# OpenDrift/opendrift

Measured on NVIDIA H100. Metric: particle-steps/sec (RK4, 10M particles/GPU, 512x512x50 field), higher is better.
Workload: dtype f64

## Files before the change

include/odcuda.h:

```cpp
#ifndef ODCUDA_H
#define ODCUDA_H

#include <stdint.h>

#ifdef __cplusplus
extern "C" {
#endif

typedef struct od_ctx od_ctx;

enum od_status {
    OD_OK = 0,
    OD_ERR_CUDA = -1,
    OD_ERR_ARG = -2,
    OD_ERR_STATE = -3,
    OD_ERR_NOMEM = -4
};

enum od_scheme { OD_EULER = 0, OD_RK2 = 1, OD_RK4 = 2 };

enum od_time_mode {
    OD_T_LERP = 0,
    OD_T_FIRST = 1,
    OD_T_SECOND = 2,
// ... 8 lines not shown
                       OD_INTERP_NEAREST = 32  };

#define OD_MAX_LEVELS 128
#define OD_ABI_VERSION 1

int od_abi_version(void);

int od_create(int device, od_ctx** out);
void od_destroy(od_ctx* ctx);
const char* od_last_error(od_ctx* ctx);
int od_set_stream(od_ctx* ctx, void* cuda_stream);
int od_sync(od_ctx* ctx);
enum od_option { OD_OPT_TILE = 1, OD_OPT_SPEC = 2 };
int od_set_option(od_ctx* ctx, int option, int value);
int od_device_sm_count(od_ctx* ctx);

#define OD_PROJ_STERE_SPHERE 1
#define OD_PROJ_MERC 2
#define OD_PROJ_LCC 3
#define OD_PROJ_STERE_ELLPS 4
#define OD_PROJ_OB_TRAN 5
typedef struct od_proj_desc {
    int32_t kind;
    int32_t has_lat_ts;
    double a;
    double lat_0, lon_0, lat_ts;
    double k_0, x_0, y_0;
    double es;
    double lat_1, lat_2;
} od_proj_desc;

typedef struct od_group_desc {
    int32_t ncomp;
    int32_t nx, ny, nz;
    int32_t lon_mode;
    int32_t n_slots;
    int32_t wrap_x;
    int32_t global_x;
    double x0, xspan, y0, yspan;
    double xmin, xmax, ymin, ymax;
    float fallback[2];
    od_proj_desc proj;
    int32_t rotate_vectors;
    int32_t pad_;
} od_group_desc;

#define OD_MAX_GROUPS 64
int od_group_define(od_ctx* ctx, int group, const od_group_desc* desc, const double* h_z_levels);
int od_group_free(od_ctx* ctx, int group);
int od_group_upload(od_ctx* ctx, int group, int slot, int comp, const float* src, int src_is_device);
int od_group_fill_nan(od_ctx* ctx, int group, int slot, int comp, int max_iterations, int64_t* h_remaining);
int od_group_slot_ptr(od_ctx* ctx, int group, int slot, int comp, float** d_out);
int od_group_touch(od_ctx* ctx, int group, int slot);
int od_group_set_window(od_ctx* ctx, int group, const od_group_desc* window);
int od_bbox(od_ctx* ctx, int64_t n, const double* d_lon, const double* d_lat, double* h_out4);
int od_group_set_fallback(od_ctx* ctx, int group, float fallback0, float fallback1);

typedef struct od_time_sample {
    int32_t slot_a, slot_b;
    int32_t mode;
    int32_t pad_;
    double w;
} od_time_sample;

int od_interp(od_ctx* ctx, int group, const od_time_sample* ts, int64_t n,
              const double* d_lon, const double* d_lat, const void* d_z, int flags,
              void* d_out0, void* d_out1);

int od_geod_fwd(od_ctx* ctx, int64_t n, double* d_lon, double* d_lat,
                const double* d_az_deg, const double* d_dist_m);

int od_update_positions(od_ctx* ctx, int64_t n, double* d_lon, double* d_lat,
                        const void* d_xvel, const void* d_yvel, int vel_f64,
                        const int32_t* d_moving, double dt);

#define OD_MATH_EXACT 0
#define OD_MATH_FAST 1
#define OD_MATH_SERIES 2

typedef struct od_advect_args {
    int32_t scheme;
    int32_t group_uv;
    od_time_sample t_start;
    od_time_sample t_mid;
    od_time_sample t_end;
    double dt;
    int64_t n;
    double* d_lon;
    double* d_lat;
    const void* d_z;
    const void* d_factor;
    int32_t factor_f64;
    int32_t pos_f32;
    const int32_t* d_moving;
    const float* d_k1_u;
    const float* d_k1_v;
    double truncate_below;
    float* d_env_u;
    float* d_env_v;
    int32_t z_f64;
    int32_t pad3_;
    const double* d_noise_cur;
    int32_t noise_kinds;
    int32_t fast;
    int32_t n_chain;
    int32_t chain_group[2];
// ... 335 lines not shown
```

opendrift_b200/_lib.py:

```python
import ctypes as C
import os

_HERE = os.path.dirname(os.path.abspath(__file__))
LIB_PATH = os.environ.get('ODCUDA_LIB') or os.path.join(_HERE, 'libodcuda.so')

OD_EULER, OD_RK2, OD_RK4 = 0, 1, 2
OD_T_LERP, OD_T_FIRST, OD_T_SECOND, OD_T_MISSING = 0, 1, 2, 3
OD_LON_0_360, OD_LON_PM180 = 0, 1
OD_OPT_TILE = 1
OD_OPT_SPEC = 2
OD_MATH_EXACT, OD_MATH_FAST, OD_MATH_SERIES = 0, 1, 2
OD_MIX_ENVIRONMENT, OD_MIX_LARGE1994, OD_MIX_SUNDBY1983, OD_MIX_CONSTANT = 0, 1, 2, 3
OD_MAX_LEVELS = 128
OD_MAX_GROUPS = 64
OD_MAX_CHAIN = 2
SCHEMES = {'euler': OD_EULER, 'runge-kutta': OD_RK2, 'runge-kutta4': OD_RK4}


class ProjDesc(C.Structure):
    _fields_ = [('kind', C.c_int32), ('has_lat_ts', C.c_int32), ('a', C.c_double), ('lat_0', C.c_double),
                ('lon_0', C.c_double), ('lat_ts', C.c_double), ('k_0', C.c_double), ('x_0', C.c_double), ('y_0', C.c_double),
                ('es', C.c_double), ('lat_1', C.c_double), ('lat_2', C.c_double)]


# ... 102 lines not shown
                ('d_sea_floor', C.c_void_p), ('d_status', C.c_void_p), ('d_moving', C.c_void_p), ('dt', C.c_double),
                ('sea_surface_height', C.c_float), ('z_f64', C.c_int32), ('tv_f64', C.c_int32), ('seafloor_code', C.c_int32),
                ('h_n_deactivated', C.POINTER(C.c_int64))]


class BookkeepArgs(C.Structure):
    _fields_ = [('n', C.c_int64), ('d_lon', C.c_void_p), ('d_lat', C.c_void_p), ('d_z', C.c_void_p), ('d_age', C.c_void_p),
                ('d_status', C.c_void_p), ('d_moving', C.c_void_p), ('d_ids', C.c_void_p), ('dt_age', C.c_double),
                ('max_age', C.c_double), ('west', C.c_double), ('east', C.c_double), ('south', C.c_double), ('north', C.c_double),
                ('outside_code', C.c_int32), ('retired_code', C.c_int32), ('z_f64', C.c_int32), ('age_f64', C.c_int32),
                ('pos_f32', C.c_int32), ('only_deactivated', C.c_int32), ('n_total', C.c_int64), ('col', C.c_int32), ('ncols', C.c_int32),
                ('d_buf_lon', C.c_void_p), ('d_buf_lat', C.c_void_p), ('d_buf_z', C.c_void_p), ('d_buf_status', C.c_void_p),
                ('h_counts', C.POINTER(C.c_int64))]


class CoastArgs(C.Structure):
    _fields_ = [('n', C.c_int64), ('d_mask', C.c_void_p), ('d_lon', C.c_void_p), ('d_lat', C.c_void_p), ('d_z', C.c_void_p),
                ('d_age', C.c_void_p), ('d_status', C.c_void_p), ('d_moving', C.c_void_p), ('d_ids', C.c_void_p),
                ('d_prev_lon', C.c_void_p), ('d_prev_lat', C.c_void_p), ('n_total', C.c_int64), ('id_base', C.c_int32),
                ('action', C.c_int32), ('ssh', C.c_float), ('stranded_code', C.c_int32), ('seeded_code', C.c_int32), ('missing_code', C.c_int32),
                ('check_seeded', C.c_int32), ('z_f64', C.c_int32), ('age_f64', C.c_int32), ('h_counts', C.POINTER(C.c_int64))]


OD_INTERP_POS_F32, OD_INTERP_NO_FALLBACK, OD_INTERP_Z_F64, OD_INTERP_NO_ROTATE, OD_INTERP_OUT_F64, OD_INTERP_NEAREST = 1, 2, 4, 8, 16, 32
OD_PACK_MAX_COLS, OD_PACK_MAX_WORLD = 16, 64


class PackArgs(C.Structure):
    _fields_ = [('n', C.c_int64), ('d_lon', C.c_void_p), ('h_bounds', C.POINTER(C.c_double)), ('world', C.c_int32), ('ncols', C.c_int32),
                ('d_cols', C.c_void_p * OD_PACK_MAX_COLS), ('col_bytes', C.c_int32 * OD_PACK_MAX_COLS), ('rec_bytes', C.c_int32),
                ('pad_', C.c_int32), ('d_records', C.c_void_p), ('d_perm', C.c_void_p), ('h_counts', C.POINTER(C.c_int64))]


OD_PROJ_STERE_SPHERE = 1
OD_PROJ_MERC, OD_PROJ_LCC, OD_PROJ_STERE_ELLPS, OD_PROJ_OB_TRAN = 2, 3, 4, 5
OD_ANALYTIC_DOUBLE_GYRE = 1

_P = C.c_void_p
SYMBOLS = {
    'od_abi_version': (C.c_int, []),
    'od_create': (C.c_int, [C.c_int, C.POINTER(_P)]),
    'od_destroy': (None, [_P]),
    'od_last_error': (C.c_char_p, [_P]),
    'od_set_stream': (C.c_int, [_P, _P]),
    'od_sync': (C.c_int, [_P]),
    'od_set_option': (C.c_int, [_P, C.c_int, C.c_int]),
    'od_device_sm_count': (C.c_int, [_P]),
    'od_group_define': (C.c_int, [_P, C.c_int, C.POINTER(GroupDesc), C.POINTER(C.c_double)]),
    'od_group_free': (C.c_int, [_P, C.c_int]),
    'od_group_upload': (C.c_int, [_P, C.c_int, C.c_int, C.c_int, _P, C.c_int]),
    'od_group_fill_nan': (C.c_int, [_P, C.c_int, C.c_int, C.c_int, C.c_int, C.POINTER(C.c_int64)]),
    'od_group_slot_ptr': (C.c_int, [_P, C.c_int, C.c_int, C.c_int, C.POINTER(_P)]),
    'od_group_touch': (C.c_int, [_P, C.c_int, C.c_int]),
    'od_group_set_fallback': (C.c_int, [_P, C.c_int, C.c_float, C.c_float]),
    'od_group_set_window': (C.c_int, [_P, C.c_int, C.POINTER(GroupDesc)]),
    'od_bbox': (C.c_int, [_P, C.c_int64, _P, _P, C.POINTER(C.c_double)]),
    'od_interp': (C.c_int, [_P, C.c_int, C.POINTER(TimeSample), C.c_int64, _P, _P, _P, C.c_int, _P, _P]),
    'od_geod_fwd': (C.c_int, [_P, C.c_int64, _P, _P, _P, _P]),
    'od_update_positions': (C.c_int, [_P, C.c_int64, _P, _P, _P, _P, C.c_int, _P, C.c_double]),
    'od_advect_current': (C.c_int, [_P, C.POINTER(AdvectArgs)]),
    'od_advect_current_host': (C.c_int, [_P, C.POINTER(AdvectArgs), C.POINTER(HostIO)]),
    'od_step_oceandrift_host': (C.c_int, [_P, C.POINTER(StepArgs), C.POINTER(HostIO)]),
    'od_step_oceandrift': (C.c_int, [_P, C.POINTER(StepArgs)]),
    'od_leeway_step': (C.c_int, [_P, C.POINTER(LeewayArgs)]),
    'od_analytic_interp': (C.c_int, [_P, C.POINTER(AnalyticDesc), C.c_double, C.c_int64, _P, _P, C.c_int, _P, _P]),
    'od_history_scatter': (C.c_int, [_P, C.POINTER(HistoryArgs)]),
    'od_analytic_advect': (C.c_int, [_P, C.POINTER(AnalyticDesc), C.POINTER(AnalyticAdvectArgs)]),
    'od_minmax_f32': (C.c_int, [_P, C.c_int64, _P, _P, C.POINTER(C.c_float), C.POINTER(C.c_float)]),
    'od_stokes_drift': (C.c_int, [_P, C.POINTER(StokesArgs)]),
    'od_stokes_parameterised': (C.c_int, [_P, C.c_int64, _P, _P, _P, C.c_int32, _P, C.c_int32, _P, _P, _P]),
    'od_vertical_mixing': (C.c_int, [_P, C.POINTER(MixArgs)]),
    'od_vertical_mixing_settle': (C.c_int, [_P, C.POINTER(MixArgs), _P, _P, C.POINTER(C.c_int64)]),
    'od_resuspend': (C.c_int, [_P, C.c_int64, _P, _P, C.c_float, _P, _P, C.c_int32]),
    'od_ship_step': (C.c_int, [_P, C.c_int64, _P, _P, _P, _P, _P, _P, _P, _P, _P, C.c_int32, C.c_int32, C.c_int32, C.c_int32, C.c_int32,
                               C.c_int32, C.c_float, C.c_int32, C.c_double, C.POINTER(C.c_int32)]),
    'od_plast_step': (C.c_int, [_P, C.c_int64, _P, _P, _P, _P, C.c_int32, _P, _P, _P, C.c_int32, _P, _P, C.c_uint64, C.c_int32, _P, C.c_int32,
                                C.c_int32, _P, _P, _P, C.c_int32, C.c_double, C.c_double, C.POINTER(C.c_int32)]),
    'od_larval_develop': (C.c_int, [_P, C.c_int64, _P, _P, _P, C.c_int32, _P, C.c_int32, _P, C.c_int32, _P, C.c_int32, _P, C.c_int32, _P,
                                    C.c_int32, C.c_int32, _P, C.c_double, C.POINTER(C.c_int32)]),
    'od_larval_migrate': (C.c_int, [_P, C.c_int64, _P, C.c_int32, _P, C.c_int32, _P, C.c_int32, C.c_double, C.c_double, C.c_double]),
    'od_vertical_buoyancy': (C.c_int, [_P, C.POINTER(BuoyancyArgs)]),
    'od_bookkeeping': (C.c_int, [_P, C.POINTER(BookkeepArgs)]),
    'od_coastline': (C.c_int, [_P, C.POINTER(CoastArgs)]),
    'od_store_previous': (C.c_int, [_P, C.c_int64, _P, _P, _P, C.c_int32, C.c_int64, _P, _P]),
    'od_store_previous_env': (C.c_int, [_P, C.c_int64, _P, _P, _P, C.c_int32, C.c_double, C.c_int32, C.c_int64, _P, _P]),
    'od_vertical_advection_corrected': (C.c_int, [_P, C.c_int64, _P, C.c_int32, _P, _P, _P, _P, C.c_float, _P, C.c_int32,
                                                  C.c_double]),
    'od_pack_by_owner': (C.c_int, [_P, C.POINTER(PackArgs)]),
    'od_unpack_records': (C.c_int, [_P, C.c_int64, _P, C.c_int32, C.POINTER(_P), C.POINTER(C.c_int32), C.c_int32]),
    'od_sort_by_cell': (C.c_int, [_P, C.c_int, C.c_int64, _P, _P, _P, _P]),
    'od_partition_active': (C.c_int, [_P, C.c_int64, _P, _P, C.POINTER(C.c_int64)]),
    'od_permute': (C.c_int, [_P, C.c_int64, _P, _P, _P, C.c_int]),
    'od_unpermute': (C.c_int, [_P, C.c_int64, _P, _P, _P, C.c_int]),
    'od_launch_count': (C.c_int64, [_P]),
}

_lib = None


def load():
    global _lib
    if _lib is not None:
        return _lib
    if not os.path.exists(LIB_PATH):
        raise RuntimeError(
            'opendrift_b200: %s is missing. This package has no CPU fallback; build the CUDA '
# ... 12 lines not shown
```

opendrift_b200/csrc/od_ctx.cuh:

```cuda
#pragma once
#include <cuda.h>
#include <cuda_runtime.h>
#include <stdint.h>
#include <string>
#include <vector>

#include "../../include/odcuda.h"
#include "od_advect.cuh"
#include "od_analytic.cuh"

using namespace od;

#define OD_PAIR_CACHE 4
#ifndef OD_BLOCK
#define OD_BLOCK 128
#endif
#ifndef OD_STEP_MINB
#define OD_STEP_MINB 8
#endif
#ifndef OD_SPEC_MINB
#define OD_SPEC_MINB 6
#endif

#define OD_TILE_BX 48
#define OD_TILE_BY 8
#define OD_TILE_BZ 2
#define OD_TILE_HALO 2

struct PairEntry {
    CUtensorMap tmap;
    bool tmap_ok = false;
    float* tex = nullptr;
    int slot_a = -1, slot_b = -1;
    uint64_t ver_a = 0, ver_b = 0;
    uint64_t last_use = 0;
};

struct Group {
    bool defined = false;
    od_group_desc desc;
    std::vector<float*> slots;
    std::vector<uint64_t> version;
    double* d_zs = nullptr;
    double* d_zy = nullptr;
    double* d_zl = nullptr;
    double* d_mxs = nullptr;
    double* d_mxy = nullptr;
    std::vector<double> h_levels;
    double zmin = 0, zmax = 0;
    PairEntry pairs[OD_PAIR_CACHE];
    size_t capacity = 0;
    size_t cells() const { return (size_t)desc.nx * desc.ny * desc.nz; }
};

struct od_ctx {
    int device = 0;
    cudaStream_t stream = nullptr;
    std::string err;
    Group groups[OD_MAX_GROUPS];
    int64_t launches = 0;
    uint64_t tick = 0;
    int sm_count = 0;
    int32_t* d_keys = nullptr;
    int32_t* d_bins = nullptr;
    int64_t keys_cap = 0, bins_cap = 0;
    int32_t* d_tilesums = nullptr;
    int64_t tiles_cap = 0;
    unsigned* d_red = nullptr;
    unsigned long long* d_bbox = nullptr;
    unsigned* d_cnt = nullptr;
    float* d_fill = nullptr;
    unsigned* d_fillcnt = nullptr;
    int coop_fill_blocks = -1;
    int64_t fill_cap = 0;
    int tile = 0;
    int spec = 1;
    cudaStream_t hstream[3] = {nullptr, nullptr, nullptr};
    cudaEvent_t hready = nullptr;
    char* hbuf = nullptr;
    int64_t hbuf_cap = 0;
};

static inline int fail(od_ctx* c, int code, const char* what, cudaError_t e = cudaSuccess) {
    if (c) {
        c->err = what;
        if (e != cudaSuccess) {
            c->err += ": ";
            c->err += cudaGetErrorString(e);
// ... 32 lines not shown
```

opendrift_b200/csrc/od_kernels.cu:

```cuda
#include <cuda.h>
#include <cuda_runtime.h>
#include <cooperative_groups.h>
#include <stdint.h>
#include <stdio.h>
#include <stdlib.h>
#include <string.h>
#include <string>
#include <vector>

#include "../../include/odcuda.h"
#include "od_advect.cuh"
#include "od_mix.cuh"
#include "od_stokes.cuh"
#include "od_leeway.cuh"
#include "od_ship.cuh"
#include "od_plast.cuh"
#include "od_larval.cuh"
#include "od_analytic.cuh"
#include "od_history.cuh"
#include "od_bookkeep.cuh"
#include "od_sealevel.cuh"
#include "od_ctx.cuh"

extern "C" int od_abi_version(void) { return OD_ABI_VERSION; }

extern "C" int od_create(int device, od_ctx** out) {
    if (!out) return OD_ERR_ARG;
    *out = nullptr;
    int count = 0;
    if (cudaGetDeviceCount(&count) != cudaSuccess || device < 0 || device >= count) return OD_ERR_CUDA;
    if (cudaSetDevice(device) != cudaSuccess) return OD_ERR_CUDA;
    od_ctx* c = new od_ctx();
    c->device = device;
    cudaDeviceGetAttribute(&c->sm_count, cudaDevAttrMultiProcessorCount, device);
    *out = c;
    return OD_OK;
}

static void free_group(Group& g) {
    for (float* p : g.slots) if (p) cudaFree(p);
    g.slots.clear();
    g.version.clear();
    if (g.d_zs) cudaFree(g.d_zs);
    if (g.d_zy) cudaFree(g.d_zy);
    if (g.d_zl) cudaFree(g.d_zl);
    if (g.d_mxs) cudaFree(g.d_mxs);
    if (g.d_mxy) cudaFree(g.d_mxy);
    g.d_zs = g.d_zy = g.d_zl = g.d_mxs = g.d_mxy = nullptr;
    g.h_levels.clear();
    for (auto& p : g.pairs) {
        if (p.tex) cudaFree(p.tex);
        p = PairEntry();
    }
    g.defined = false;
}

extern "C" void od_destroy(od_ctx* ctx) {
    if (!ctx) return;
    cudaSetDevice(ctx->device);
    for (auto& g : ctx->groups) free_group(g);
    if (ctx->d_keys) cudaFree(ctx->d_keys);
    if (ctx->d_bins) cudaFree(ctx->d_bins);
    if (ctx->d_red) cudaFree(ctx->d_red);
    if (ctx->d_bbox) cudaFree(ctx->d_bbox);
    if (ctx->d_cnt) cudaFree(ctx->d_cnt);
    if (ctx->d_fill) cudaFree(ctx->d_fill);
    if (ctx->d_fillcnt) cudaFree(ctx->d_fillcnt);
    if (ctx->d_tilesums) cudaFree(ctx->d_tilesums);
    if (ctx->hbuf) cudaFree(ctx->hbuf);
    for (int k = 0; k < 3; ++k)
        if (ctx->hstream[k]) cudaStreamDestroy(ctx->hstream[k]);
    if (ctx->hready) cudaEventDestroy(ctx->hready);
    delete ctx;
}

extern "C" const char* od_last_error(od_ctx* ctx) { return ctx ? ctx->err.c_str() : "null context"; }

extern "C" int od_set_stream(od_ctx* ctx, void* s) {
    if (!ctx) return OD_ERR_ARG;
    ctx->stream = (cudaStream_t)s;
    return OD_OK;
}

extern "C" int od_set_option(od_ctx* ctx, int option, int value) {
    if (!ctx) return OD_ERR_ARG;
    if (option == OD_OPT_TILE) { ctx->tile = value ? 1 : 0; return OD_OK; }
    if (option == OD_OPT_SPEC) { ctx->spec = value ? 1 : 0; return OD_OK; }
    return fail(ctx, OD_ERR_ARG, "od_set_option: unknown option");
}

extern "C" int od_sync(od_ctx* ctx) {
    if (!ctx) return OD_ERR_ARG;
    CK(cudaStreamSynchronize(ctx->stream));
    return OD_OK;
}

extern "C" int od_device_sm_count(od_ctx* ctx) { return ctx ? ctx->sm_count : 0; }
extern "C" int64_t od_launch_count(od_ctx* ctx) { return ctx ? ctx->launches : 0; }

extern "C" int od_group_define(od_ctx* ctx, int group, const od_group_desc* d, const double* h_z) {
    if (!ctx || !d || group < 0 || group >= OD_MAX_GROUPS) return fail(ctx, OD_ERR_ARG, "od_group_define: bad group");
    if (d->ncomp < 1 || d->ncomp > 2 || d->nx < 2 || d->ny < 2 || d->nz < 1 || d->nz > OD_MAX_LEVELS ||
        d->n_slots < 2 || d->n_slots > 64)
        return fail(ctx, OD_ERR_ARG, "od_group_define: bad shape");
// ... 260 lines not shown
        }
        if (still) atomicAdd(&cnt[it + 1], still);
        grid.sync();
        for (int64_t i = first; i < cells; i += stride) a[i] = tmp[i];
        grid.sync();
    }
}

__global__ void __launch_bounds__(OD_BLOCK) pack_pair2_kernel(const float* __restrict__ a0, const float* __restrict__ a1,
                                                               const float* __restrict__ b0, const float* __restrict__ b1,
                                                               float4* __restrict__ tex, int64_t cells) {
    int64_t i = (int64_t)blockIdx.x * blockDim.x + threadIdx.x;
    const int64_t stride = (int64_t)gridDim.x * blockDim.x;
    for (; i < cells; i += stride) tex[i] = make_float4(a0[i], a1[i], b0[i], b1[i]);
}

__global__ void __launch_bounds__(OD_BLOCK) pack_pair1_kernel(const float* __restrict__ a0, const float* __restrict__ b0,
                                                               float2* __restrict__ tex, int64_t cells) {
    int64_t i = (int64_t)blockIdx.x * blockDim.x + threadIdx.x;
    const int64_t stride = (int64_t)gridDim.x * blockDim.x;
    for (; i < cells; i += stride) tex[i] = make_float2(a0[i], b0[i]);
}

typedef CUresult (*od_encode_tiled_fn)(CUtensorMap*, CUtensorMapDataType, cuuint32_t, void*, const cuuint64_t*, const cuuint64_t*,
                                       const cuuint32_t*, const cuuint32_t*, CUtensorMapInterleave, CUtensorMapSwizzle,
                                       CUtensorMapL2promotion, CUtensorMapFloatOOBfill);

static od_encode_tiled_fn tensor_map_encoder() {
    static od_encode_tiled_fn fn = nullptr;
    static bool tried = false;
    if (!tried) {
        tried = true;
        void* f = nullptr;
        cudaDriverEntryPointQueryResult q;
        if (cudaGetDriverEntryPoint("cuTensorMapEncodeTiled", &f, cudaEnableDefault, &q) == cudaSuccess &&
            q == cudaDriverEntryPointSuccess)
            fn = (od_encode_tiled_fn)f;
    }
    return fn;
}

static bool make_tensor_map(const Group& g, float* tex, CUtensorMap* out) {
    od_encode_tiled_fn enc = tensor_map_encoder();
    if (!enc || g.desc.ncomp != 2) return false;
    const cuuint64_t dims[4] = {4, (cuuint64_t)g.desc.nx, (cuuint64_t)g.desc.ny, (cuuint64_t)g.desc.nz};
    const cuuint64_t strides[3] = {16, (cuuint64_t)g.desc.nx * 16, (cuuint64_t)g.desc.nx * g.desc.ny * 16};
    const cuuint32_t box[4] = {4, OD_TILE_BX, OD_TILE_BY, (cuuint32_t)(g.desc.nz < OD_TILE_BZ ? g.desc.nz : OD_TILE_BZ)};
    const cuuint32_t estr[4] = {1, 1, 1, 1};
    if (g.desc.nx < OD_TILE_BX || g.desc.ny < OD_TILE_BY) return false;
    return enc(out, CU_TENSOR_MAP_DATA_TYPE_FLOAT32, 4, tex, dims, strides, box, estr, CU_TENSOR_MAP_INTERLEAVE_NONE,
               CU_TENSOR_MAP_SWIZZLE_NONE, CU_TENSOR_MAP_L2_PROMOTION_L2_128B, CU_TENSOR_MAP_FLOAT_OOB_FILL_NONE) == CUDA_SUCCESS;
}

static int resolve_pair(od_ctx* ctx, int group, const od_time_sample& ts, PairRef* out) {
    Group& g = ctx->groups[group];
    const int nc = g.desc.ncomp;
    if (ts.mode == OD_T_MISSING) {
        out->tex = nullptr; out->mode = OD_T_MISSING; out->pad_ = 0; out->w = 0.0;
        return OD_OK;
    }
    int sa = ts.slot_a, sb = ts.slot_b;
    if (ts.mode == OD_T_FIRST) sb = (sb < 0 || sb >= g.desc.n_slots) ? sa : sb;
    if (ts.mode == OD_T_SECOND) sa = (sa < 0 || sa >= g.desc.n_slots) ? sb : sa;
    if (sa < 0 || sa >= g.desc.n_slots || sb < 0 || sb >= g.desc.n_slots || ts.mode < 0 || ts.mode > 2)
        return fail(ctx, OD_ERR_ARG, "bad time sample");
    out->w = ts.w;
    out->pad_ = 0;
    if (ts.mode != OD_T_LERP) {
        const int need = ts.mode == OD_T_FIRST ? sa : sb;
        for (auto& p : g.pairs) {
            if (!p.tex) continue;
            if (p.slot_a == need && p.ver_a == g.version[need]) { out->tex = p.tex; out->mode = OD_T_FIRST; p.last_use = ++ctx->tick; return OD_OK; }
            if (p.slot_b == need && p.ver_b == g.version[need]) { out->tex = p.tex; out->mode = OD_T_SECOND; p.last_use = ++ctx->tick; return OD_OK; }
        }
    }
    for (auto& p : g.pairs) {
        if (p.tex && p.slot_a == sa && p.slot_b == sb && p.ver_a == g.version[sa] && p.ver_b == g.version[sb]) {
            out->tex = p.tex;
            out->mode = ts.mode;
            p.last_use = ++ctx->tick;
            return OD_OK;
        }
    }
    PairEntry* victim = &g.pairs[0];
    for (auto& p : g.pairs) {
        if (!p.tex) { victim = &p; break; }
        if (p.last_use < victim->last_use) victim = &p;
    }
    if (!victim->tex) {
        CK(cudaMalloc(&victim->tex, g.capacity * sizeof(float) * 2 * nc));
        victim->tmap_ok = make_tensor_map(g, victim->tex, &victim->tmap);
        for (auto& p : g.pairs) {
            if (p.tex) continue;
            if (cudaMalloc(&p.tex, g.capacity * sizeof(float) * 2 * nc) != cudaSuccess) {
                p.tex = nullptr;
                cudaGetLastError();
                break;
            }
            p.tmap_ok = make_tensor_map(g, p.tex, &p.tmap);
        }
    }
    const int64_t cells = (int64_t)g.cells();
    int blocks = (int)((cells + OD_BLOCK - 1) / OD_BLOCK);
    const int cap = ctx->sm_count * 8;
    if (blocks > cap) blocks = cap;
    if (nc == 2)
        pack_pair2_kernel<<<blocks, OD_BLOCK, 0, ctx->stream>>>(g.slots[(size_t)sa * 2], g.slots[(size_t)sa * 2 + 1],
                                                                g.slots[(size_t)sb * 2], g.slots[(size_t)sb * 2 + 1],
                                                                (float4*)victim->tex, cells);
    else
        pack_pair1_kernel<<<blocks, OD_BLOCK, 0, ctx->stream>>>(g.slots[sa], g.slots[sb], (float2*)victim->tex, cells);
    CK(cudaGetLastError());
    ctx->launches++;
    victim->slot_a = sa;
    victim->slot_b = sb;
    victim->ver_a = g.version[sa];
    victim->ver_b = g.version[sb];
    victim->last_use = ++ctx->tick;
    out->tex = victim->tex;
    out->mode = ts.mode;
    return OD_OK;
}

static GroupGeom make_geom(const Group& g) {
    GroupGeom q;
    memset(&q, 0, sizeof(q));
    q.nx = g.desc.nx; q.ny = g.desc.ny; q.nz = g.desc.nz; q.ncomp = g.desc.ncomp;
    q.lon_mode = g.desc.lon_mode;
    q.wrap = g.desc.wrap_x ? 1 : 0;
    q.glob = (g.desc.global_x || g.desc.wrap_x) ? 1 : 0;
    q.x0 = g.desc.x0; q.xspan = g.desc.xspan; q.y0 = g.desc.y0; q.yspan = g.desc.yspan;
    q.xmin = g.desc.xmin; q.xmax = g.desc.xmax; q.ymin = g.desc.ymin; q.ymax = g.desc.ymax;
    q.nxm1 = (double)(g.desc.nx - 1 + q.wrap); q.nym1 = (double)(g.desc.ny - 1);
    q.inv_dx = q.nxm1 / q.xspan; q.inv_dy = q.nym1 / q.yspan;
    q.rxspan = div_rn_reciprocal(q.xspan); q.ryspan = div_rn_reciprocal(q.yspan);
    q.zmin = g.zmin; q.zmax = g.zmax;
    q.fallback[0] = g.desc.fallback[0]; q.fallback[1] = g.desc.fallback[1];
    q.zs = g.d_zs; q.zy = g.d_zy;
    if (g.desc.proj.kind != 0 && proj_from_desc(&g.desc.proj, &q.proj) == 0) {
        q.proj_kind = g.desc.proj.kind;
        q.rotate = g.desc.rotate_vectors ? 1 : 0;
        q.rot_delta = q.proj_kind == OD_PROJ_OB_TRAN ? kObTranRotDelta : 10.0;
    }
    return q;
}

struct InterpParams {
    GroupGeom g;
    PairRef pr;
    int64_t n;
    const double* lon;
    const double* lat;
    const void* z;
    void* out0;
    void* out1;
    int pos_f32, z_f64;
    int out_f64, nearest;
};

template <bool PROJ>
__global__ void __launch_bounds__(OD_BLOCK) interp_kernel(const InterpParams p) {
    __shared__ LevelsSmem lv;
    if (p.g.nz > 1) load_levels(lv, p.g);
    __syncthreads();
    const int64_t i = (int64_t)blockIdx.x * blockDim.x + threadIdx.x;
    if (i >= p.n) return;
    const double z = (p.z && p.g.nz > 1) ? (p.z_f64 ? ((const double*)p.z)[i] : (double)((const float*)p.z)[i]) : 0.0;
    const VertW vw = vert_weights(p.g, (const double*)lv.zs, (const double*)lv.zy, z, p.z_f64 == 0);
    if (p.nearest) {
        const float r = sample1_nearest(p.g, p.pr, p.lon[i], p.lat[i], p.pos_f32 != 0);
        if (p.out0) { if (p.out_f64) ((double*)p.out0)[i] = (double)r; else ((float*)p.out0)[i] = r; }
// ... 157 lines not shown
__device__ __forceinline__ unsigned f2ord(float f) {
    const unsigned u = __float_as_uint(f);
    return (u & 0x80000000u) ? ~u : (u | 0x80000000u);
}
static float ord2f(unsigned u) {
    u = (u & 0x80000000u) ? (u & 0x7fffffffu) : ~u;
    float f;
    memcpy(&f, &u, 4);
    return f;
}

__global__ void __launch_bounds__(256) minmax_kernel(int64_t n, const float* __restrict__ a, const float* __restrict__ b,
                                                     unsigned* __restrict__ out) {
    unsigned lo = 0xffffffffu, hi = 0u;
    for (int64_t i = (int64_t)blockIdx.x * blockDim.x + threadIdx.x; i < n; i += (int64_t)gridDim.x * blockDim.x) {
        const float v = b ? __fadd_rn(a[i], b[i]) : a[i];
        if (v == v) {
            const unsigned o = f2ord(v);
            lo = min(lo, o);
            hi = max(hi, o);
        }
    }
    for (int o = 16; o > 0; o >>= 1) {
        lo = min(lo, __shfl_xor_sync(0xffffffffu, lo, o));
        hi = max(hi, __shfl_xor_sync(0xffffffffu, hi, o));
    }
    if ((threadIdx.x & 31) == 0) {
        atomicMin(&out[0], lo);
        atomicMax(&out[1], hi);
    }
}

__global__ void __launch_bounds__(256) stokes_tab_kernel(const StokesTabParams p) {
    for (int64_t i = (int64_t)blockIdx.x * blockDim.x + threadIdx.x; i < p.n; i += (int64_t)gridDim.x * blockDim.x)
        stokes_tab_one(p, i);
}

struct SortParams {
    GroupGeom g;
    int64_t n;
    const double* lon;
    const double* lat;
    const float* z;
    int tile, ntx, nty;
};

template <bool PROJ>
__global__ void __launch_bounds__(OD_BLOCK) cell_key_kernel(const SortParams p, int32_t* __restrict__ keys,
                                                             int32_t* __restrict__ bins) {
    __shared__ LevelsSmem lv;
    if (p.g.nz > 1) load_levels(lv, p.g);
    __syncthreads();
    const int64_t i = (int64_t)blockIdx.x * blockDim.x + threadIdx.x;
    if (i >= p.n) return;
    const HorizW h = PROJ ? horiz_weights_h(p.g, p.lon[i], p.lat[i], false) : horiz_weights(p.g, p.lon[i], p.lat[i], false);
    int key = 0;
    if (h.valid) {
        const int iy = h.i00 / p.g.nx, ix = h.i00 - iy * p.g.nx;
        const VertW vw = vert_weights(p.g, (const double*)lv.zs, (const double*)lv.zy, (p.z && p.g.nz > 1) ? (double)p.z[i] : 0.0);
        key = 1 + (vw.ia * p.nty + iy / p.tile) * p.ntx + ix / p.tile;
    }
    keys[i] = key;
    atomicAdd(&bins[key], 1);
}

__global__ void __launch_bounds__(1024) scan_bins_kernel(int32_t* __restrict__ bins, int nbins) {
    __shared__ int32_t warp_sums[32];
    __shared__ int32_t carry;
    if (threadIdx.x == 0) carry = 0;
    __syncthreads();
    for (int base = 0; base < nbins; base += 1024) {
        const int i = base + threadIdx.x;
        int v = i < nbins ? bins[i] : 0;
        int x = v;
        for (int o = 1; o < 32; o <<= 1) {
            int y = __shfl_up_sync(0xffffffffu, x, o);
            if ((threadIdx.x & 31) >= o) x += y;
        }
        if ((threadIdx.x & 31) == 31) warp_sums[threadIdx.x >> 5] = x;
        __syncthreads();
        if (threadIdx.x < 32) {
            int s = warp_sums[threadIdx.x];
            for (int o = 1; o < 32; o <<= 1) {
                int y = __shfl_up_sync(0xffffffffu, s, o);
                if (threadIdx.x >= o) s += y;
            }
            warp_sums[threadIdx.x] = s;
        }
        __syncthreads();
        const int warp_off = (threadIdx.x >> 5) ? warp_sums[(threadIdx.x >> 5) - 1] : 0;
        const int incl = x + warp_off + carry;
        if (i < nbins) bins[i] = incl - v;
        __syncthreads();
        if (threadIdx.x == 1023) carry = incl;
        __syncthreads();
    }
}

#define OD_SCAN_TILE 4096
__global__ void __launch_bounds__(1024) scan_tiles_kernel(int32_t* __restrict__ bins, int nbins, int32_t* __restrict__ tile_sums) {
    __shared__ int32_t warp_sums[32];
    const int base = blockIdx.x * OD_SCAN_TILE + threadIdx.x * 4;
    int v[4];
#pragma unroll
    for (int k = 0; k < 4; ++k) v[k] = base + k < nbins ? bins[base + k] : 0;
    const int mine = v[0] + v[1] + v[2] + v[3];
    int x = mine;
    for (int o = 1; o < 32; o <<= 1) {
        int y = __shfl_up_sync(0xffffffffu, x, o);
        if ((threadIdx.x & 31) >= o) x += y;
    }
    if ((threadIdx.x & 31) == 31) warp_sums[threadIdx.x >> 5] = x;
    __syncthreads();
    if (threadIdx.x < 32) {
        int t = warp_sums[threadIdx.x];
        for (int o = 1; o < 32; o <<= 1) {
            int y = __shfl_up_sync(0xffffffffu, t, o);
            if (threadIdx.x >= o) t += y;
        }
        warp_sums[threadIdx.x] = t;
    }
    __syncthreads();
    int run = x - mine + ((threadIdx.x >> 5) ? warp_sums[(threadIdx.x >> 5) - 1] : 0);
#pragma unroll
    for (int k = 0; k < 4; ++k) {
        if (base + k < nbins) bins[base + k] = run;
        run += v[k];
    }
    if (threadIdx.x == 1023) tile_sums[blockIdx.x] = run;
}

__global__ void __launch_bounds__(1024) add_tile_offsets_kernel(int32_t* __restrict__ bins, int nbins, const int32_t* __restrict__ tile_sums) {
    const int off = tile_sums[blockIdx.x];
    const int base = blockIdx.x * OD_SCAN_TILE + threadIdx.x * 4;
#pragma unroll
    for (int k = 0; k < 4; ++k)
        if (base + k < nbins) bins[base + k] += off;
}

static int scan_exclusive(od_ctx* ctx, int32_t* bins, int nbins) {
    if (nbins <= 2 * OD_SCAN_TILE) {
        scan_bins_kernel<<<1, 1024, 0, ctx->stream>>>(bins, nbins);
        ctx->launches++;
        return OD_OK;
    }
    const int ntiles = (nbins + OD_SCAN_TILE - 1) / OD_SCAN_TILE;
    const int rc = grow(ctx, (void**)&ctx->d_tilesums, &ctx->tiles_cap, ntiles, sizeof(int32_t));
    if (rc) return rc;
    scan_tiles_kernel<<<ntiles, 1024, 0, ctx->stream>>>(bins, nbins, ctx->d_tilesums);
    scan_bins_kernel<<<1, 1024, 0, ctx->stream>>>(ctx->d_tilesums, ntiles);
    add_tile_offsets_kernel<<<ntiles, 1024, 0, ctx->stream>>>(bins, nbins, ctx->d_tilesums);
    ctx->launches += 3;
    return OD_OK;
}

__global__ void __launch_bounds__(OD_BLOCK) scatter_perm_kernel(int64_t n, const int32_t* __restrict__ keys,
                                                                 int32_t* __restrict__ bins, int32_t* __restrict__ perm) {
    const int64_t i = (int64_t)blockIdx.x * blockDim.x + threadIdx.x;
    if (i >= n) return;
    const int pos = atomicAdd(&bins[keys[i]], 1);
    perm[pos] = (int32_t)i;
}

#define OD_PART_BLOCK 256
__global__ void __launch_bounds__(OD_PART_BLOCK) partition_count_kernel(int64_t n, const int32_t* __restrict__ status,
                                                                        int32_t* __restrict__ block_keep) {
    const int64_t i = (int64_t)blockIdx.x * blockDim.x + threadIdx.x;
    const int keep = (i < n && status[i] == 0) ? 1 : 0;
    const int c = __syncthreads_count(keep);
    if (threadIdx.x == 0) block_keep[blockIdx.x] = c;
}

__global__ void __launch_bounds__(OD_PART_BLOCK) partition_scatter_kernel(int64_t n, const int32_t* __restrict__ status,
                                                                          const int32_t* __restrict__ block_keep_excl,
                                                                          int64_t n_keep, int32_t* __restrict__ perm) {
    __shared__ int warp_keep[OD_PART_BLOCK / 32];
    const int64_t i = (int64_t)blockIdx.x * blockDim.x + threadIdx.x;
    const bool valid = i < n;
    const int keep = (valid && status[i] == 0) ? 1 : 0;
    const unsigned ballot = __ballot_sync(0xffffffffu, keep);
    const int lane = threadIdx.x & 31, warp = threadIdx.x >> 5;
    const int rank_in_warp = __popc(ballot & ((1u << lane) - 1u));
    if (lane == 0) warp_keep[warp] = __popc(ballot);
    __syncthreads();
    int before = 0;
    for (int w = 0; w < warp; ++w) before += warp_keep[w];
    const int64_t keep_base = block_keep_excl[blockIdx.x];
    const int64_t first = (int64_t)blockIdx.x * blockDim.x;
    if (!valid) return;
    const int local_keep_rank = before + rank_in_warp;
    const int local_index = (int)(i - first);
    if (keep) perm[keep_base + local_keep_rank] = (int32_t)i;
    else perm[n_keep + (first - keep_base) + (local_index - local_keep_rank)] = (int32_t)i;
}

template <typename T>
__global__ void __launch_bounds__(OD_BLOCK) permute_kernel(int64_t n, const int32_t* __restrict__ perm,
                                                            const T* __restrict__ src, T* __restrict__ dst, int inverse) {
    const int64_t k = (int64_t)blockIdx.x * blockDim.x + threadIdx.x;
    if (k >= n) return;
    if (inverse) dst[perm[k]] = src[k];
    else dst[k] = src[perm[k]];
}

#define OD_PACK_BLOCK 256

struct PackParams {
    int64_t n;
    const double* lon;
    int world, ncols, rec_bytes, nblocks;
    double bounds[OD_PACK_MAX_WORLD + 1];
    const unsigned char* cols[OD_PACK_MAX_COLS];
    int col_bytes[OD_PACK_MAX_COLS];
    int col_off[OD_PACK_MAX_COLS];
// ... 1146 lines not shown
```

opendrift_b200/engine.py:

```python
import ctypes as C
import gc
import weakref
from bisect import bisect_left

import numpy as np

from . import _lib
from ._lib import (GroupDesc, TimeSample, AdvectArgs, StepArgs, MixArgs, StokesArgs, LeewayArgs, OD_T_LERP, OD_T_FIRST,
                   OD_T_MISSING, SCHEMES)


def _seconds(t, t0):
    return (t - t0).total_seconds() if hasattr(t - t0, 'total_seconds') else float(t - t0)


def bracket(times, t):
    if len(times) == 1:
        return 0, None, 0.0
    if t < times[0] or t > times[-1]:
        return None
    ib = max(0, bisect_left(times, t) - 1)
    if times[ib + 1] == t:
        ib += 1
    tb = times[ib]
# ... 24 lines not shown
            cur[st, 0, 1] = np.random.normal(0, cur_std, n)
        if cur_uniform > 0:
            cur[st, 1, 0] = np.random.uniform(-cur_uniform, cur_uniform, n)
            cur[st, 1, 1] = np.random.uniform(-cur_uniform, cur_uniform, n)
        if st == 0 and with_wind and wind_std > 0:
            wind = np.stack([np.random.normal(0, wind_std, n), np.random.normal(0, wind_std, n)])
    return cur, kinds, wind


def _ptr(t):
    if t is None:
        return None
    return C.c_void_p(t.data_ptr())


SHIP_ELEMENTS = ('length', 'height', 'draft', 'beam', 'wind_drag_coeff', 'water_drag_coeff')
SHIP_ENV = ('x_sea_water_velocity', 'y_sea_water_velocity', 'x_wind', 'y_wind', 'hs', 'period', 'stokes_x', 'stokes_y',
            'land_binary_mask')


def grid_geometry(lon, lat):
    lon = np.asarray(lon, dtype=np.float32)
    lat = np.asarray(lat, dtype=np.float32)
    xmin, xmax = float(lon.min()), float(lon.max())
    dx = float(lon[1] - lon[0])
    glob = (xmin - 2 * dx <= 0 and xmax + 2 * dx >= 360) or (xmin - 2 * dx <= -180 and xmax + 2 * dx >= 180)
    periodic = bool(glob) and abs(len(lon) * dx - 360.0) < 1e-3 * dx
    x_last = np.float32(lon[-1] + np.float32(dx)) if periodic else lon[-1]
    return {'lon_mode': _lib.OD_LON_PM180 if xmin < 0 else _lib.OD_LON_0_360, 'wrap_x': 1 if periodic else 0, 'global_x': 1 if glob else 0,
            'global_coverage': bool(glob),
            'x0': float(lon[0]), 'xspan': float(np.float32(x_last - lon[0])),
            'y0': float(lat[0]), 'yspan': float(np.float32(lat[-1] - lat[0])),
            'xmin': xmin, 'xmax': xmax, 'ymin': float(lat.min()), 'ymax': float(lat.max())}


class FieldGroup:

    def __init__(self, engine, gid, lon, lat, z, ncomp, times, supplier, fallback, n_slots=3,
                 names=None, proj=None, lon_0to360=False, rotate=False):
        self.engine, self.gid, self.ncomp = engine, gid, ncomp
        self.lon = np.asarray(lon, dtype=np.float32)
        self.lat = np.asarray(lat, dtype=np.float32)
        self.z = None if z is None else np.asarray(z, dtype=np.float64)
        self.times = list(times)
        self.supplier = supplier
        self.names = names
        self.n_slots = n_slots
        self.freed = False
        self.fill_nan = 10
        self.resident = [None] * n_slots
        self.use = [0] * n_slots
        self.ready = [None] * n_slots
        self.prefetch_on = True
        self._tick = 0
        d = GroupDesc()
        d.ncomp, d.nx, d.ny = ncomp, len(self.lon), len(self.lat)
        d.nz = 1 if self.z is None else len(self.z)
        d.n_slots = n_slots
        geo = grid_geometry(self.lon, self.lat)
        if proj is not None:
            geo.update(lon_mode=_lib.OD_LON_0_360 if lon_0to360 else _lib.OD_LON_PM180, wrap_x=0, global_x=0, global_coverage=False)
            d.proj = proj
            d.rotate_vectors = 1 if (rotate and ncomp == 2) else 0
        d.lon_mode, d.wrap_x, d.global_x = geo['lon_mode'], geo['wrap_x'], geo['global_x']
        d.x0, d.xspan, d.y0, d.yspan = geo['x0'], geo['xspan'], geo['y0'], geo['yspan']
        d.xmin, d.xmax, d.ymin, d.ymax = geo['xmin'], geo['xmax'], geo['ymin'], geo['ymax']
        self.global_coverage, self.periodic = geo['global_coverage'], bool(geo['wrap_x'])
        fb = list(fallback) + [float('nan')] * (2 - len(fallback))
        d.fallback[0] = float('nan') if fb[0] is None else fb[0]
        d.fallback[1] = float('nan') if fb[1] is None else fb[1]
        self.desc = d
        zl = None
        if self.z is not None:
            zl = (C.c_double * len(self.z))(*self.z)
        engine._check(engine.lib.od_group_define(engine.ctx, gid, C.byref(d), zl))

    def set_window(self, lon, lat):
        lon = np.asarray(lon, dtype=np.float32)
        lat = np.asarray(lat, dtype=np.float32)
        d = self.desc
        d.nx, d.ny = len(lon), len(lat)
        d.x0, d.xspan = float(lon[0]), float(np.float32(lon[-1] - lon[0]))
        d.y0, d.yspan = float(lat[0]), float(np.float32(lat[-1] - lat[0]))
        self.lon, self.lat = lon, lat
        self.engine.order_after_copies()
        self.engine._check(self.engine.lib.od_group_set_window(self.engine.ctx, self.gid, C.byref(d)))
        self.resident = [None] * self.n_slots
        self.ready = [None] * self.n_slots

    def set_fallback(self, fallback):
        fb = list(fallback) + [None] * (2 - len(fallback))
        fb = [float('nan') if v is None else float(v) for v in fb]
        self.desc.fallback[0], self.desc.fallback[1] = fb[0], fb[1]
        self.engine._check(self.engine.lib.od_group_set_fallback(self.engine.ctx, self.gid, fb[0], fb[1]))

    def __del__(self):
        try:
            self.engine.free_group(self)
        except Exception:
            pass

    def _victim(self, pinned):
        cand = [s for s in range(self.n_slots) if self.resident[s] not in pinned or self.resident[s] is None]
        if not cand:
            return None
        return min(cand, key=lambda k: (self.resident[k] is not None, self.use[k]))

    def _load(self, ti, s):
        eng = self.engine
        d = eng.dist
        eng.order_after_copies()
        if d is None or d.rank == d.src:
            for c in range(self.ncomp):
                eng.upload(self.gid, s, c, self.supplier(ti, c))
                if self.fill_nan:
                    eng.fill_nan(self.gid, s, c, self.fill_nan)
        if d is not None:
            for c in range(self.ncomp):
                d.broadcast(eng.slot_tensor(self, s, c))
            if d.rank != d.src:
                eng.touch(self.gid, s)
            d.slabs_broadcast += 1

    def slot_of(self, ti, pinned=()):
        self._tick += 1
        if ti in self.resident:
            s = self.resident.index(ti)
            self.use[s] = self._tick
            if self.ready[s] is not None:
                self.engine.wait_event(self.ready[s])
                self.ready[s] = None
            return s
        s = self._victim(pinned)
        assert s is not None, 'no free ring slot'
        self._load(ti, s)
        self.resident[s] = ti
        self.ready[s] = None
        self.use[s] = self._tick
        return s

    def prefetch(self, ti, pinned=()):
        if not self.prefetch_on or ti < 0 or ti >= len(self.times) or ti in self.resident:
            return False
        s = self._victim(pinned)
        if s is None or self.resident[s] in pinned:
            return False
        eng = self.engine
        if not eng.begin_copy_stream():
            return False
        try:
            self._load(ti, s)
            self.ready[s] = eng.end_copy_stream()
        except Exception:
            eng.end_copy_stream()
            raise
        self.resident[s] = ti
        self.use[s] = 0
        return True

    def sample(self, t, pinned=()):
        ts = TimeSample()
        br = bracket(self.times, t)
        if br is None:
            ts.mode = OD_T_MISSING
            return ts, ()
        ib, ia, w = br
        if ia is None:
            ts.slot_a = self.slot_of(ib, pinned)
            ts.slot_b = -1
            ts.mode = OD_T_FIRST
            return ts, (ib,)
        sa = self.slot_of(ib, tuple(pinned) + (ia,))
        sb = self.slot_of(ia, tuple(pinned) + (ib,))
        ts.slot_a, ts.slot_b, ts.mode, ts.w = sa, sb, OD_T_LERP, w
        if self.n_slots > 2 and len(self.times) > 2:
            nxt = ia + 1 if self.engine.direction >= 0 else ib - 1
            self.prefetch(nxt, tuple(pinned) + (ib, ia))
        return ts, (ib, ia)


def bind_process_to_gpu_numa(device_index):
    import os
    import subprocess
    info = {'device': int(device_index), 'bound': False}
    try:
        bus = subprocess.run(['nvidia-smi', '-i', str(device_index), '--query-gpu=pci.bus_id', '--format=csv,noheader'],
                             capture_output=True, text=True, timeout=20).stdout.strip().lower()
        if not bus:
            return info
        if len(bus.split(':')[0]) == 8:
            bus = bus[4:]
        node_path = '/sys/bus/pci/devices/%s/numa_node' % bus
        node = int(open(node_path).read().strip())
        info['pci_bus_id'], info['numa_node'] = bus, node
        if node < 0:
            return info
        cpus = set()
        for part in open('/sys/devices/system/node/node%d/cpulist' % node).read().strip().split(','):
            a, _, b = part.partition('-')
            cpus.update(range(int(a), int(b or a) + 1))
        cpus &= os.sched_getaffinity(0)
        if cpus:
            os.sched_setaffinity(0, cpus)
            info['bound'], info['cpus'] = True, len(cpus)
# ... 103 lines not shown
        assert status is not None and moving is not None and status.dtype == torch.int32
        a.d_status, a.d_moving_out, a.seafloor_code = status.data_ptr(), moving.data_ptr(), int(seafloor_code)
        a.h_n_deactivated = C.pointer(nd)
    return a, z_out, nd


class Engine:
    def __init__(self, device=0):
        import torch
        if not torch.cuda.is_available():
            raise RuntimeError('opendrift_b200 needs a CUDA device (H100, sm_90a); there is no CPU fallback')
        self.torch = torch
        self.lib = _lib.load()
        self.device = torch.device('cuda', device)
        torch.cuda.set_device(self.device)
        ctx = C.c_void_p()
        rc = self.lib.od_create(device, C.byref(ctx))
        if rc != 0:
            raise RuntimeError('od_create failed (%d)' % rc)
        self.ctx = ctx
        self.use_stream(torch.cuda.current_stream(self.device))
        self.groups = weakref.WeakValueDictionary()
        self.math_mode = _lib.OD_MATH_SERIES
        self.dist = None
        self.direction = 1
        self._main_stream = torch.cuda.current_stream(self.device)
        self._copy_stream = None
        self._in_copy = False

    def wait_event(self, ev):
        self.torch.cuda.current_stream(self.device).wait_event(ev)

    def order_after_copies(self):
        ev = getattr(self, '_last_copy_event', None)
        if ev is not None and not self._in_copy:
            self.wait_event(ev)
            self._last_copy_event = None

    def begin_copy_stream(self):
        if self._in_copy:
            return False
        torch = self.torch
        if self._copy_stream is None:
            self._copy_stream = torch.cuda.Stream(device=self.device)
        self._main_stream = torch.cuda.current_stream(self.device)
        self._copy_stream.wait_stream(self._main_stream)
        self._ctx_mgr = torch.cuda.stream(self._copy_stream)
        self._ctx_mgr.__enter__()
        self.use_stream(self._copy_stream)
        self._in_copy = True
        return True

    def end_copy_stream(self):
        ev = self.torch.cuda.Event()
        ev.record(self._copy_stream)
        self._ctx_mgr.__exit__(None, None, None)
        self.use_stream(self._main_stream)
        self._in_copy = False
        self._last_copy_event = ev
        return ev

    def enable_distributed(self, src=0, group=None):
        import torch.distributed as dist
        if dist.is_available() and dist.is_initialized() and dist.get_world_size(group) > 1:
            self.dist = DistContext(dist, dist.get_rank(group), dist.get_world_size(group), src, group)
        return self.dist

    def touch(self, gid, slot):
        self._check(self.lib.od_group_touch(self.ctx, gid, slot))

    def close(self):
        if getattr(self, 'ctx', None):
            self.lib.od_destroy(self.ctx)
            self.ctx = None

    def __del__(self):
        try:
            self.close()
        except Exception:
            pass

    def _check(self, rc):
        if rc != 0:
            raise RuntimeError('libodcuda: %s (status %d)' % (self.lib.od_last_error(self.ctx).decode(), rc))

    def use_stream(self, stream):
        self._check(self.lib.od_set_stream(self.ctx, C.c_void_p(stream.cuda_stream)))

    def set_tile(self, on):
        self._check(self.lib.od_set_option(self.ctx, _lib.OD_OPT_TILE, 1 if on else 0))

    def set_spec(self, on):
        self._check(self.lib.od_set_option(self.ctx, _lib.OD_OPT_SPEC, 1 if on else 0))

    def sync(self):
        self._check(self.lib.od_sync(self.ctx))

    def launches(self):
        return int(self.lib.od_launch_count(self.ctx))

    def to_device(self, a, dtype=None):
        t = self.torch.as_tensor(np.ascontiguousarray(a))
        if dtype is not None:
            t = t.to(dtype)
        return t.to(self.device, non_blocking=True)

# ... 609 lines not shown
```

Measured before the change: 8.549 billion.

## Prebuild next time-pair texture on copy stream and warp-aggregate binning atomics

Adds od_group_prepare_pair so the packed pair texture for the next time bracket is built on the prefetch copy stream right after the new slot loads. A per-pair event orders later consumers after that build, so the main stream no longer stalls packing at time-step boundaries. The keying and scatter kernels also use __match_any_sync to merge same-key atomics within a warp. This adds event bookkeeping and uses one fewer pair cache entry for speculative work, which risks evicting a pair that is still needed.

```diff
diff --git a/include/odcuda.h b/include/odcuda.h
--- a/include/odcuda.h
+++ b/include/odcuda.h
@@ -84,6 +84,7 @@
 int od_group_fill_nan(od_ctx* ctx, int group, int slot, int comp, int max_iterations, int64_t* h_remaining);
 int od_group_slot_ptr(od_ctx* ctx, int group, int slot, int comp, float** d_out);
 int od_group_touch(od_ctx* ctx, int group, int slot);
+int od_group_prepare_pair(od_ctx* ctx, int group, int slot_a, int slot_b);
 int od_group_set_window(od_ctx* ctx, int group, const od_group_desc* window);
 int od_bbox(od_ctx* ctx, int64_t n, const double* d_lon, const double* d_lat, double* h_out4);
 int od_group_set_fallback(od_ctx* ctx, int group, float fallback0, float fallback1);
diff --git a/opendrift_b200/_lib.py b/opendrift_b200/_lib.py
--- a/opendrift_b200/_lib.py
+++ b/opendrift_b200/_lib.py
@@ -178,6 +178,7 @@
     'od_group_fill_nan': (C.c_int, [_P, C.c_int, C.c_int, C.c_int, C.c_int, C.POINTER(C.c_int64)]),
     'od_group_slot_ptr': (C.c_int, [_P, C.c_int, C.c_int, C.c_int, C.POINTER(_P)]),
     'od_group_touch': (C.c_int, [_P, C.c_int, C.c_int]),
+    'od_group_prepare_pair': (C.c_int, [_P, C.c_int, C.c_int, C.c_int]),
     'od_group_set_fallback': (C.c_int, [_P, C.c_int, C.c_float, C.c_float]),
     'od_group_set_window': (C.c_int, [_P, C.c_int, C.POINTER(GroupDesc)]),
     'od_bbox': (C.c_int, [_P, C.c_int64, _P, _P, C.POINTER(C.c_double)]),
diff --git a/opendrift_b200/csrc/od_ctx.cuh b/opendrift_b200/csrc/od_ctx.cuh
--- a/opendrift_b200/csrc/od_ctx.cuh
+++ b/opendrift_b200/csrc/od_ctx.cuh
@@ -34,6 +34,8 @@
     int slot_a = -1, slot_b = -1;
     uint64_t ver_a = 0, ver_b = 0;
     uint64_t last_use = 0;
+    cudaEvent_t ready = nullptr;
+    bool pending = false;
 };
 
 struct Group {
diff --git a/opendrift_b200/csrc/od_kernels.cu b/opendrift_b200/csrc/od_kernels.cu
--- a/opendrift_b200/csrc/od_kernels.cu
+++ b/opendrift_b200/csrc/od_kernels.cu
@@ -50,6 +50,7 @@
     g.h_levels.clear();
     for (auto& p : g.pairs) {
         if (p.tex) cudaFree(p.tex);
+        if (p.ready) cudaEventDestroy(p.ready);
         p = PairEntry();
     }
     g.defined = false;
@@ -416,41 +417,19 @@
                CU_TENSOR_MAP_SWIZZLE_NONE, CU_TENSOR_MAP_L2_PROMOTION_L2_128B, CU_TENSOR_MAP_FLOAT_OOB_FILL_NONE) == CUDA_SUCCESS;
 }
 
-static int resolve_pair(od_ctx* ctx, int group, const od_time_sample& ts, PairRef* out) {
-    Group& g = ctx->groups[group];
+static int order_after_build(od_ctx* ctx, PairEntry& p) {
+    if (!p.pending) return OD_OK;
+    if (cudaEventQuery(p.ready) == cudaSuccess) {
+        p.pending = false;
+        return OD_OK;
+    }
+    cudaGetLastError();
+    CK(cudaStreamWaitEvent(ctx->stream, p.ready, 0));
+    return OD_OK;
+}
+
+static int build_pair(od_ctx* ctx, Group& g, int sa, int sb, PairEntry* victim, int max_blocks) {
     const int nc = g.desc.ncomp;
-    if (ts.mode == OD_T_MISSING) {
-        out->tex = nullptr; out->mode = OD_T_MISSING; out->pad_ = 0; out->w = 0.0;
-        return OD_OK;
-    }
-    int sa = ts.slot_a, sb = ts.slot_b;
-    if (ts.mode == OD_T_FIRST) sb = (sb < 0 || sb >= g.desc.n_slots) ? sa : sb;
-    if (ts.mode == OD_T_SECOND) sa = (sa < 0 || sa >= g.desc.n_slots) ? sb : sa;
-    if (sa < 0 || sa >= g.desc.n_slots || sb < 0 || sb >= g.desc.n_slots || ts.mode < 0 || ts.mode > 2)
-        return fail(ctx, OD_ERR_ARG, "bad time sample");
-    out->w = ts.w;
-    out->pad_ = 0;
-    if (ts.mode != OD_T_LERP) {
-        const int need = ts.mode == OD_T_FIRST ? sa : sb;
-        for (auto& p : g.pairs) {
-            if (!p.tex) continue;
-            if (p.slot_a == need && p.ver_a == g.version[need]) { out->tex = p.tex; out->mode = OD_T_FIRST; p.last_use = ++ctx->tick; return OD_OK; }
-            if (p.slot_b == need && p.ver_b == g.version[need]) { out->tex = p.tex; out->mode = OD_T_SECOND; p.last_use = ++ctx->tick; return OD_OK; }
-        }
-    }
-    for (auto& p : g.pairs) {
-        if (p.tex && p.slot_a == sa && p.slot_b == sb && p.ver_a == g.version[sa] && p.ver_b == g.version[sb]) {
-            out->tex = p.tex;
-            out->mode = ts.mode;
-            p.last_use = ++ctx->tick;
-            return OD_OK;
-        }
-    }
-    PairEntry* victim = &g.pairs[0];
-    for (auto& p : g.pairs) {
-        if (!p.tex) { victim = &p; break; }
-        if (p.last_use < victim->last_use) victim = &p;
-    }
     if (!victim->tex) {
         CK(cudaMalloc(&victim->tex, g.capacity * sizeof(float) * 2 * nc));
         victim->tmap_ok = make_tensor_map(g, victim->tex, &victim->tmap);
@@ -464,10 +443,12 @@
             p.tmap_ok = make_tensor_map(g, p.tex, &p.tmap);
         }
     }
+    int rc = order_after_build(ctx, *victim);
+    if (rc) return rc;
+    victim->pending = false;
     const int64_t cells = (int64_t)g.cells();
     int blocks = (int)((cells + OD_BLOCK - 1) / OD_BLOCK);
-    const int cap = ctx->sm_count * 8;
-    if (blocks > cap) blocks = cap;
+    if (blocks > max_blocks) blocks = max_blocks;
     if (nc == 2)
         pack_pair2_kernel<<<blocks, OD_BLOCK, 0, ctx->stream>>>(g.slots[(size_t)sa * 2], g.slots[(size_t)sa * 2 + 1],
                                                                 g.slots[(size_t)sb * 2], g.slots[(size_t)sb * 2 + 1],
@@ -481,6 +462,84 @@
     victim->ver_a = g.version[sa];
     victim->ver_b = g.version[sb];
     victim->last_use = ++ctx->tick;
+    return OD_OK;
+}
+
+extern "C" int od_group_prepare_pair(od_ctx* ctx, int group, int slot_a, int slot_b) {
+    int rc = check_slot(ctx, group, slot_a, 0);
+    if (rc) return rc;
+    rc = check_slot(ctx, group, slot_b, 0);
+    if (rc) return rc;
+    CK(cudaSetDevice(ctx->device));
+    Group& g = ctx->groups[group];
+    PairEntry* newest = nullptr;
+    for (auto& p : g.pairs) {
+        if (p.tex && p.slot_a == slot_a && p.slot_b == slot_b && p.ver_a == g.version[slot_a] && p.ver_b == g.version[slot_b])
+            return OD_OK;
+        if (p.tex && (!newest || p.last_use > newest->last_use)) newest = &p;
+    }
+    PairEntry* victim = nullptr;
+    for (auto& p : g.pairs) {
+        if (&p == newest) continue;
+        if (!p.tex) { victim = &p; break; }
+        if (!victim || p.last_use < victim->last_use) victim = &p;
+    }
+    if (!victim) return OD_OK;
+    rc = build_pair(ctx, g, slot_a, slot_b, victim, ctx->sm_count);
+    if (rc) return rc;
+    if (!victim->ready) CK(cudaEventCreateWithFlags(&victim->ready, cudaEventDisableTiming));
+    CK(cudaEventRecord(victim->ready, ctx->stream));
+    victim->pending = true;
+    return OD_OK;
+}
+
+static int resolve_pair(od_ctx* ctx, int group, const od_time_sample& ts, PairRef* out) {
+    Group& g = ctx->groups[group];
+    if (ts.mode == OD_T_MISSING) {
+        out->tex = nullptr; out->mode = OD_T_MISSING; out->pad_ = 0; out->w = 0.0;
+        return OD_OK;
+    }
+    int sa = ts.slot_a, sb = ts.slot_b;
+    if (ts.mode == OD_T_FIRST) sb = (sb < 0 || sb >= g.desc.n_slots) ? sa : sb;
+    if (ts.mode == OD_T_SECOND) sa = (sa < 0 || sa >= g.desc.n_slots) ? sb : sa;
+    if (sa < 0 || sa >= g.desc.n_slots || sb < 0 || sb >= g.desc.n_slots || ts.mode < 0 || ts.mode > 2)
+        return fail(ctx, OD_ERR_ARG, "bad time sample");
+    out->w = ts.w;
+    out->pad_ = 0;
+    if (ts.mode != OD_T_LERP) {
+        const int need = ts.mode == OD_T_FIRST ? sa : sb;
+        for (int pass = 0; pass < 2; ++pass) {
+            for (auto& p : g.pairs) {
+                if (!p.tex) continue;
+                if (pass == 0 && p.pending && cudaEventQuery(p.ready) != cudaSuccess) { cudaGetLastError(); continue; }
+                int mode = -1;
+                if (p.slot_a == need && p.ver_a == g.version[need]) mode = OD_T_FIRST;
+                else if (p.slot_b == need && p.ver_b == g.version[need]) mode = OD_T_SECOND;
+                if (mode < 0) continue;
+                const int rc = order_after_build(ctx, p);
+                if (rc) return rc;
+                out->tex = p.tex; out->mode = mode; p.last_use = ++ctx->tick;
+                return OD_OK;
+            }
+        }
+    }
+    for (auto& p : g.pairs) {
+        if (p.tex && p.slot_a == sa && p.slot_b == sb && p.ver_a == g.version[sa] && p.ver_b == g.version[sb]) {
+            const int rc = order_after_build(ctx, p);
+            if (rc) return rc;
+            out->tex = p.tex;
+            out->mode = ts.mode;
+            p.last_use = ++ctx->tick;
+            return OD_OK;
+        }
+    }
+    PairEntry* victim = &g.pairs[0];
+    for (auto& p : g.pairs) {
+        if (!p.tex) { victim = &p; break; }
+        if (p.last_use < victim->last_use) victim = &p;
+    }
+    const int rc = build_pair(ctx, g, sa, sb, victim, ctx->sm_count * 8);
+    if (rc) return rc;
     out->tex = victim->tex;
     out->mode = ts.mode;
     return OD_OK;
@@ -744,16 +803,19 @@
     if (p.g.nz > 1) load_levels(lv, p.g);
     __syncthreads();
     const int64_t i = (int64_t)blockIdx.x * blockDim.x + threadIdx.x;
-    if (i >= p.n) return;
-    const HorizW h = PROJ ? horiz_weights_h(p.g, p.lon[i], p.lat[i], false) : horiz_weights(p.g, p.lon[i], p.lat[i], false);
-    int key = 0;
-    if (h.valid) {
-        const int iy = h.i00 / p.g.nx, ix = h.i00 - iy * p.g.nx;
-        const VertW vw = vert_weights(p.g, (const double*)lv.zs, (const double*)lv.zy, (p.z && p.g.nz > 1) ? (double)p.z[i] : 0.0);
-        key = 1 + (vw.ia * p.nty + iy / p.tile) * p.ntx + ix / p.tile;
-    }
-    keys[i] = key;
-    atomicAdd(&bins[key], 1);
+    int key = -1;
+    if (i < p.n) {
+        const HorizW h = PROJ ? horiz_weights_h(p.g, p.lon[i], p.lat[i], false) : horiz_weights(p.g, p.lon[i], p.lat[i], false);
+        key = 0;
+        if (h.valid) {
+            const int iy = h.i00 / p.g.nx, ix = h.i00 - iy * p.g.nx;
+            const VertW vw = vert_weights(p.g, (const double*)lv.zs, (const double*)lv.zy, (p.z && p.g.nz > 1) ? (double)p.z[i] : 0.0);
+            key = 1 + (vw.ia * p.nty + iy / p.tile) * p.ntx + ix / p.tile;
+        }
+        keys[i] = key;
+    }
+    const unsigned peers = __match_any_sync(0xffffffffu, key);
+    if (key >= 0 && (threadIdx.x & 31) == __ffs(peers) - 1) atomicAdd(&bins[key], __popc(peers));
 }
 
 __global__ void __launch_bounds__(1024) scan_bins_kernel(int32_t* __restrict__ bins, int nbins) {
@@ -849,9 +911,13 @@
 __global__ void __launch_bounds__(OD_BLOCK) scatter_perm_kernel(int64_t n, const int32_t* __restrict__ keys,
                                                                  int32_t* __restrict__ bins, int32_t* __restrict__ perm) {
     const int64_t i = (int64_t)blockIdx.x * blockDim.x + threadIdx.x;
-    if (i >= n) return;
-    const int pos = atomicAdd(&bins[keys[i]], 1);
-    perm[pos] = (int32_t)i;
+    const int key = i < n ? keys[i] : -1;
+    const unsigned peers = __match_any_sync(0xffffffffu, key);
+    const int lane = threadIdx.x & 31, leader = __ffs(peers) - 1;
+    int base = 0;
+    if (key >= 0 && lane == leader) base = atomicAdd(&bins[key], __popc(peers));
+    base = __shfl_sync(0xffffffffu, base, leader);
+    if (key >= 0) perm[base + __popc(peers & ((1u << lane) - 1u))] = (int32_t)i;
 }
 
 #define OD_PART_BLOCK 256
diff --git a/opendrift_b200/engine.py b/opendrift_b200/engine.py
--- a/opendrift_b200/engine.py
+++ b/opendrift_b200/engine.py
@@ -100,6 +100,7 @@
         self.use = [0] * n_slots
         self.ready = [None] * n_slots
         self.prefetch_on = True
+        self.ahead_pair = None
         self._tick = 0
         d = GroupDesc()
         d.ncomp, d.nx, d.ny = ncomp, len(self.lon), len(self.lat)
@@ -198,6 +199,9 @@
             return False
         try:
             self._load(ti, s)
+            nb = ti - 1 if eng.direction >= 0 else ti + 1
+            if nb in self.resident:
+                self.ahead_pair = (self.resident.index(nb), s) if nb < ti else (s, self.resident.index(nb))
             self.ready[s] = eng.end_copy_stream()
         except Exception:
             eng.end_copy_stream()
@@ -407,6 +411,11 @@
         return True
 
     def end_copy_stream(self):
+        for g in list(self.groups.values()):
+            if g.ahead_pair is not None:
+                sa, sb = g.ahead_pair
+                g.ahead_pair = None
+                self._check(self.lib.od_group_prepare_pair(self.ctx, g.gid, sa, sb))
         ev = self.torch.cuda.Event()
         ev.record(self._copy_stream)
         self._ctx_mgr.__exit__(None, None, None)
```

After: 8.852 billion (median of 6 runs). +3.5%, better.
